# RIKEN-RCCS/GEMMul8

Measured on AMD Instinct MI355X. Metric: emulated DGEMM TFLOPS (N=8192, moduli=14), higher is better.
Workload: dtype int8

## Files before the change

### gemmul8_amd/__init__.py

```python
import ctypes as C
import os

_HERE = os.path.dirname(os.path.abspath(__file__))
LIB_PATH = os.path.join(_HERE, "lib", "libgemmul8.so")

S, D, Cx, Z = 0, 1, 2, 3
INT8, FP8 = 0, 1
OPS = {"N": 0, "T": 1, "C": 2}
UPLO = {"L": 0, "U": 1}
SIDE = {"L": 0, "R": 1}
DIAG = {"N": 0, "U": 1}


class Layout(C.Structure):
    _fields_ = [
        ("kp", C.c_size_t), ("mp", C.c_size_t), ("num_mat", C.c_size_t), ("parts", C.c_size_t),
        ("sizeA", C.c_size_t), ("sizeB", C.c_size_t), ("sizeC", C.c_size_t),
        ("A_lo", C.c_void_p), ("B_lo", C.c_void_p),
        ("part_strideA", C.c_size_t), ("part_strideB", C.c_size_t),
        ("A_bound", C.c_void_p), ("B_bound", C.c_void_p),
        ("sftA", C.c_void_p), ("sftB", C.c_void_p),
        ("C_mid", C.c_void_p), ("scratch", C.c_void_p), ("scratch_bytes", C.c_size_t),
        ("lo_format", C.c_size_t),
    ]


_lib = None

EXPORTS = ["gemmul8_version", "gemmul8_work_size", "gemmul8_gemm", "gemmul8_get_layout", "gemmul8_scale",
           "gemmul8_scale_bounds", "gemmul8_scale_finish", "gemmul8_lowprec_gemm", "gemmul8_crt", "gemmul8_set_fp8_bound_mode", "gemmul8_set_nonfinite_mode",
           "gemmul8_hook_would_emulate", "gemmul8_reload_knobs", "gemmul8_abi_version", "gemmul8_layout_bytes", "gemmul8_syrk", "gemmul8_herk", "gemmul8_syr2k",
           "gemmul8_symm", "gemmul8_hemm", "gemmul8_her2k", "gemmul8_trmm", "gemmul8_trsm", "gemmul8_trsm_work_size", "gemmul8_trsm_leaf"]

ABI_VERSION = 7


def _bind_hip_runtime():
    try:
        import torch
    except Exception:
        pass
    path = None
    with open("/proc/self/maps") as f:
        for line in f:
            if "libamdhip64" in line:
                path = line.split()[-1]
                break
# ... 77 lines not shown
    L.gemmul8_trmm.argtypes = [C.c_void_p, C.c_int, C.c_int, C.c_int, C.c_int, C.c_int, C.c_int, C.c_size_t, C.c_size_t, C.c_void_p, C.c_void_p, C.c_size_t,
                               C.c_void_p, C.c_size_t, C.c_void_p, C.c_size_t, C.c_uint, C.c_int, C.c_void_p, C.POINTER(C.c_double)]
    L.gemmul8_trsm.restype = C.c_int
    L.gemmul8_trsm.argtypes = [C.c_void_p, C.c_int, C.c_int, C.c_int, C.c_int, C.c_int, C.c_int, C.c_size_t, C.c_size_t, C.c_void_p, C.c_void_p, C.c_size_t,
                               C.c_void_p, C.c_size_t, C.c_uint, C.c_int, C.c_void_p, C.POINTER(C.c_double)]
    L.gemmul8_trsm_work_size.restype = C.c_size_t
    L.gemmul8_trsm_work_size.argtypes = [C.c_int, C.c_int, C.c_int, C.c_size_t, C.c_size_t, C.c_uint]
    L.gemmul8_trsm_leaf.restype = C.c_int
    L.gemmul8_trsm_leaf.argtypes = []
    L.gemmul8_set_fp8_bound_mode.restype = C.c_int
    L.gemmul8_set_fp8_bound_mode.argtypes = [C.c_int]
    L.gemmul8_set_nonfinite_mode.restype = C.c_int
    L.gemmul8_set_nonfinite_mode.argtypes = [C.c_int]
    L.gemmul8_hook_would_emulate.restype = C.c_int
    L.gemmul8_hook_would_emulate.argtypes = [C.c_int, C.c_int, C.c_size_t, C.c_size_t, C.c_size_t, C.c_uint, C.c_int, C.c_size_t]
    L.gemmul8_reload_knobs.restype = None
    L.gemmul8_reload_knobs.argtypes = []
    L.gemmul8_add_f64.restype = C.c_int
    L.gemmul8_add_f64.argtypes = [C.c_void_p, C.c_void_p, C.c_void_p, C.c_size_t]
    L.gemmul8_add_row_bias.restype = C.c_int
    L.gemmul8_add_row_bias.argtypes = [C.c_void_p, C.c_int, C.c_size_t, C.c_size_t, C.c_void_p, C.c_size_t, C.c_void_p]
    return L


NONFINITE_REFERENCE, NONFINITE_IEEE = 0, 1


def set_nonfinite_mode(mode):
    prev = lib().gemmul8_set_nonfinite_mode(int(mode))
    if prev < 0:
# ... 308 lines not shown
```

### gemmul8_amd/csrc/oz2_driver.hip

```cpp
#include <hip/hip_runtime.h>
#include <stdint.h>
#include <stdio.h>
#include <stdlib.h>
#include <string.h>

#include <algorithm>

#include <atomic>
#include <mutex>

#include "../../include/gemmul8_c.h"
#include "oz2_gemm_common.hpp"
#include "oz2_kernels.h"
#include "oz2_knobs.hpp"

using namespace oz2;

namespace {

inline char* align256(void* p) {
    uintptr_t x = reinterpret_cast<uintptr_t>(p);
    x = (x + 255) & ~uintptr_t(255);
    return reinterpret_cast<char*>(x);
}
// ... 40 lines not shown
static Knobs parse_knobs() {
    Knobs k;
    auto num = [](const char* name, int dflt) {
        const char* s = getenv(name);
        return s && *s ? atoi(s) : dflt;
    };
    if (const char* e = getenv("GEMMUL8_EPI_NT"); e && (e[0] == '0' || e[0] == '1') && !e[1]) k.epi_nt = e[0] - '0';
    if (const int t = num("GEMMUL8_BOUND_TILE", 0); t == 128 || t == 256) k.bound_tile = t;
    if (num("GEMMUL8_CPLX_BOUND_LAUNCHES", 1) == 2) k.cplx_bound_launches = 2;
    if (const int c = num("GEMMUL8_CPLX_CHUNK", 0); c >= 1) k.cplx_chunk = c;
    if (const char* e = getenv("GEMMUL8_CRT_KERNEL")) k.crt_kernel = e[0] == 'd' ? 1 : e[0] == 'r' ? 2 : 0;
    if (const int c = num("GEMMUL8_GEMM_CUS", 0); c >= 8) k.gemm_cus = c & ~7;
    if (const char* e = getenv("GEMMUL8_FP8_FUSED"); e && e[0] == '0') k.fp8_fused = 0;
    if (const char* e = getenv("GEMMUL8_FP8_PLANES")) k.fp8_planes = e[0] == 'e' ? 1 : 0;
    if (const char* e = getenv("GEMMUL8_SCALE_FOLD"); e && e[0] == '0') k.scale_fold = 0;
    if (const char* e = getenv("GEMMUL8_BOUNDS_ONE_READ"); e && (e[0] == '0' || e[0] == '1') && !e[1]) k.bounds_one_read = e[0] - '0';
    if (const char* e = getenv("GEMMUL8_CRT_PANELS"); e && atoi(e) > 1) {
        k.crt_panels = std::min(atoi(e), 256);
        k.crt_panels_ring = e[strlen(e) - 1] == 'r';
    }
    if (const char* e = getenv("GEMMUL8_MAP_COLBLOCK"); e && *e) k.map_colblock = atoi(e) > 0 ? atoi(e) : 0;
    return k;
}
static std::atomic<const Knobs*> g_knobs{nullptr};
static std::mutex g_knobs_mtx;
void reload_knobs() {
    std::lock_guard<std::mutex> lk(g_knobs_mtx);
    g_knobs.store(new Knobs(parse_knobs()), std::memory_order_release);
}
const Knobs& knobs() {
// ... 208 lines not shown
            OZ2_HIP(launch_gemm_f8_bound_cplx(stream, 3, Ab + 2 * L->sizeA, Bb + 2 * L->sizeB, L->kp, k, m, ncols, fbuf, L->mp, rowmax,
                                              colmax + col_begin));
        } else {
            if (int rc2 = bound_gemm_i8(stream, cplx, L, m, col_end - col_begin, Ab, Bb, rowmax, colmax + col_begin)) return rc2;
        }
    }
    return GEMMUL8_OK;
}

int gemmul8_scale_bounds(void* stream_, int dtype, int backend, int op_A, int op_B, size_t m, size_t n, size_t k, const void* A,
                         size_t lda, const void* B, size_t ldb, unsigned N, size_t col_begin, size_t col_end, const gemmul8_layout* L,
                         int skipA, int skipB) {
    return scale_bounds_nf(stream_, dtype, backend, op_A, op_B, m, n, k, A, lda, B, ldb, N, col_begin, col_end, L, skipA, skipB, false);
}

struct TwinPlanes {
    int8_t* lo;
    size_t plane_stride, part_stride;
};
static int scale_finish_nf(void* stream_, int dtype, int backend, int op_A, int op_B, size_t m, size_t n, size_t k, const void* A, size_t lda,
                           const void* B, size_t ldb, unsigned N, int fastmode, unsigned t_begin, unsigned t_end, const gemmul8_layout* L, int skipA,
                           int skipB, bool nf, const TwinPlanes* twinA = nullptr, const SymSide* sym = nullptr) {
    hipStream_t stream = (hipStream_t)stream_;
    if (!L || !A || !B) return GEMMUL8_E_ARG;
    if (!moduli_ok(dtype, N) || t_end > N || t_begin > t_end) return GEMMUL8_E_NUM_MODULI;
    if (backend == kFP8 && k > 65536) return GEMMUL8_E_ARG;
    op_A = norm_op(op_A);
    op_B = norm_op(op_B);
    if (op_A < 0 || op_A > 2 || op_B < 0 || op_B > 2) return GEMMUL8_E_ARG;
    if (skipA && skipB) return GEMMUL8_OK;
    const bool cplx = is_complex(dtype);
    const bool kmajA = op_A != 0, kmajB = op_B == 0;
    const bool conjA = cplx && op_A == 2, conjB = cplx && op_B == 2;
    QuantOperand oa, ob;
    const bool f6 = backend == kFP8 && L->lo_format == 1;
    if (!skipA) oa = QuantOperand{kmajA, conjA, m, A, lda, L->sftA, (int8_t*)L->A_lo, L->sizeA, L->part_strideA, g_batch.sa, f6 ? L->mp : 0};
    if (!skipB) ob = QuantOperand{kmajB, conjB, n, B, ldb, L->sftB, (int8_t*)L->B_lo, L->sizeB, L->part_strideB, g_batch.sb, f6 ? n : 0};
    oa.nf = ob.nf = nf;
    if (twinA) oa.lo2 = twinA->lo, oa.plane_stride2 = twinA->plane_stride, oa.part_stride2 = twinA->part_stride;
    if (sym) (sym->onB ? ob : oa).sym = sym->form, (sym->onB ? ob : oa).herm = sym->herm;
    if (sym && sym->conj) (sym->onB ? ob : oa).conj = cplx;
    if (fastmode) {
        OZ2_HIP(launch_fast_shift_pair(stream, dtype, backend, N, k, oa, ob));
        if (nf) {
            FlagOperand fa, fb;
            if (!skipA) fa = FlagOperand{kmajA, m, A, lda, g_batch.sa, L->sftA};
            if (!skipB) fb = FlagOperand{kmajB, n, B, ldb, g_batch.sb, L->sftB};
            OZ2_HIP(launch_flag_pair(stream, dtype, k, fa, fb));
        }
    } else {
        int *rowmax, *colmax;
        void* amax;
        int16_t *s0A, *s0B;
        int rc = scale_scratch(L, n, &rowmax, &colmax, &amax, &s0A, &s0B);
        if (rc) return rc;
        if (t_end > t_begin && knobs().scale_fold) {
            const float log2P = backend == kINT8 ? GEMMUL8_LOG2P_INT8[N - 2] : GEMMUL8_LOG2P_FP8[N - 2];
            oa.fin_sft0 = s0A, oa.fin_max = rowmax, oa.fin_log2P = log2P;
            ob.fin_sft0 = s0B, ob.fin_max = colmax, ob.fin_log2P = log2P;
        } else {
            OZ2_HIP(launch_shift_finalize(stream, backend, N, skipA ? 0 : m, rowmax, L->sftA, skipB ? 0 : n, colmax, L->sftB, nf));
        }
    }
    OZ2_HIP(launch_quantise_pair(stream, dtype, backend, (int)t_begin, (int)t_end, k, L->kp, oa, ob));
    return GEMMUL8_OK;
}

int gemmul8_scale_finish(void* stream_, int dtype, int backend, int op_A, int op_B, size_t m, size_t n, size_t k, const void* A,
                         size_t lda, const void* B, size_t ldb, unsigned N, int fastmode, unsigned t_begin, unsigned t_end,
                         const gemmul8_layout* L, int skipA, int skipB) {
    return scale_finish_nf(stream_, dtype, backend, op_A, op_B, m, n, k, A, lda, B, ldb, N, fastmode, t_begin, t_end, L, skipA, skipB, false);
}

static int scale_nf(void* stream_, int dtype, int backend, int op_A, int op_B, size_t m, size_t n, size_t k, const void* A, size_t lda, const void* B,
                    size_t ldb, unsigned N, int fastmode, unsigned t_begin, unsigned t_end, const gemmul8_layout* L, int skipA, int skipB, bool nf,
                    const TwinPlanes* twinA = nullptr, const SymSide* sym = nullptr) {
    if (!fastmode) {
        int rc = scale_bounds_nf(stream_, dtype, backend, op_A, op_B, m, n, k, A, lda, B, ldb, N, 0, n, L, skipA, skipB, nf, sym);
        if (rc) return rc;
    }
    return scale_finish_nf(stream_, dtype, backend, op_A, op_B, m, n, k, A, lda, B, ldb, N, fastmode, t_begin, t_end, L, skipA, skipB, nf, twinA, sym);
}

int gemmul8_scale(void* stream_, int dtype, int backend, int op_A, int op_B, size_t m, size_t n, size_t k, const void* A, size_t lda,
                  const void* B, size_t ldb, unsigned N, int fastmode, unsigned t_begin, unsigned t_end, const gemmul8_layout* L,
                  int skipA, int skipB) {
    return scale_nf(stream_, dtype, backend, op_A, op_B, m, n, k, A, lda, B, ldb, N, fastmode, t_begin, t_end, L, skipA, skipB, false);
}

static int lowprec_gemm_kr(void* stream_, int dtype, int backend, size_t m, size_t n, size_t k, unsigned N, unsigned t_begin, unsigned t_end,
                           const gemmul8_layout* L, int krange) {
    hipStream_t stream = (hipStream_t)stream_;
    if (!L) return GEMMUL8_E_ARG;
    if (krange != 0 && backend != kINT8) return GEMMUL8_E_UNSUPPORTED;
    if (padding256(k) != L->kp) return GEMMUL8_E_ARG;
    if (!moduli_ok(dtype, N) || t_end > N || t_begin > t_end) return GEMMUL8_E_NUM_MODULI;
    const int8_t* A_lo = (const int8_t*)L->A_lo;
    const int8_t* B_lo = (const int8_t*)L->B_lo;
    if (backend == kFP8 && L->lo_format == 1 && n < 64) return GEMMUL8_E_ARG;
    const bool f6 = backend == kFP8 && L->lo_format == 1;
    auto launch_gemm_f8 = [f6](hipStream_t st, int which, const int8_t* A, const int8_t* B, size_t sA, size_t sB, size_t kp, size_t mm, size_t nn, int tb, int te,
                               int16_t* out, size_t ldo, size_t sO, const int16_t* r0, const int16_t* r1, size_t sR, const int16_t* rx = nullptr,
// ... 164 lines not shown
    if (dtype < 0 || dtype > 3 || backend < 0 || backend > 1) return GEMMUL8_E_ARG;
    if (!moduli_ok(dtype, N)) return GEMMUL8_E_NUM_MODULI;
    if (!alpha || !beta || !A || !B || !C || !work) return GEMMUL8_E_ARG;
    if (k > (size_t(1) << 17)) return GEMMUL8_E_ARG;
    if (m == 0 || n == 0 || k == 0) return GEMMUL8_OK;
    gemmul8_layout L;
    int rc = gemmul8_get_layout(dtype, backend, m, n, k, N, work, workA, workB, enA, enB, &L);
    if (rc) return rc;
    const bool skipA = skip_scalA && enA, skipB = skip_scalB && enB;
    Timer* T = timers_ns ? thread_timer() : nullptr;
    if (T && hipEventRecord(T->ev[0], stream) != hipSuccess) {
        (void)hipGetLastError();
        T = nullptr;
    }
    const bool nf = g_nonfinite_mode.load(std::memory_order_relaxed) == 1;
    rc = scale_nf(stream, dtype, backend, op_A, op_B, m, n, k, A, lda, B, ldb, N, fastmode, 0, N, &L, skipA, skipB, nf);
    if (rc) return rc;
    if (T) OZ2_HIP(hipEventRecord(T->ev[1], stream));
    const int P = (backend == kINT8 && !is_complex(dtype) && g_batch.batch <= 1) ? std::min<int>(knobs().crt_panels, (int)((n + 255) / 256)) : 0;
    if (P > 1) {
        const size_t tiles = (n + 255) / 256, esz = is_f32(dtype) ? 4 : 8;
        for (int p = 0; p < P; ++p) {
            const size_t c0 = std::min(n, tiles * p / P * 256), c1 = std::min(n, tiles * (p + 1) / P * 256);
            if (c1 <= c0) continue;
            gemmul8_layout Lp = L;
            Lp.B_lo = (char*)L.B_lo + c0 * L.kp;
            if (!knobs().crt_panels_ring) Lp.C_mid = (char*)L.C_mid + c0 * L.mp;
            rc = gemmul8_lowprec_gemm(stream, dtype, backend, m, c1 - c0, k, N, 0, N, &Lp);
            if (rc) return rc;
            rc = gemmul8_crt(stream, dtype, backend, N, m, c1 - c0, Lp.C_mid, L.mp, L.sizeC, L.sftA, L.sftB + c0, alpha, beta, (char*)C + c0 * ldc * esz, ldc);
            if (rc) return rc;
// ... 527 lines not shown
```

### gemmul8_amd/csrc/oz2_kernels.h

```cpp
#pragma once
#include <hip/hip_runtime.h>
#include <stddef.h>
#include <stdint.h>

#include "oz2_device.hpp"
#include "oz2_knobs.hpp"

namespace oz2 {

enum DType { kF32 = 0, kF64 = 1, kC32 = 2, kC64 = 3 };
inline bool is_complex(int dt) { return dt >= 2; }
inline bool is_f32(int dt) { return dt == kF32 || dt == kC32; }
inline size_t padding256(size_t x) { return (x + 255) / 256 * 256; }
inline unsigned planes_of(int backend, int t) { return backend == kINT8 ? 1u : (t < 6 ? 2u : 3u); }
inline unsigned num_mat(int backend, unsigned N) {
    unsigned s = 0;
    for (unsigned t = 0; t < N; ++t) s += planes_of(backend, (int)t);
    return s;
}
ModTable make_mod_table(int backend);

struct BatchCtx {
    unsigned batch = 1;
    size_t ws = 0;
// ... 63 lines not shown
    size_t xstride = 0;
    size_t f6_rows = 0;
    const int16_t* fin_sft0 = nullptr;
    const int* fin_max = nullptr;
    float fin_log2P = 0.0f;
    bool nf = false;
    int8_t* lo2 = nullptr;
    size_t plane_stride2 = 0, part_stride2 = 0;
    int sym = kSymNone;
    bool herm = false;
};
inline bool f6_planes_ok(size_t n) { return n >= 64 && knobs().fp8_planes != 1; }
hipError_t launch_fast_shift_pair(hipStream_t stream, int dtype, int backend, unsigned N, size_t k, const QuantOperand& A, const QuantOperand& B);
hipError_t launch_quantise_pair(hipStream_t stream, int dtype, int backend, int t_begin, int t_end, size_t k, size_t kp, const QuantOperand& A,
                                const QuantOperand& B);

struct Seg2Planes {
    const void* X2 = nullptr;
    size_t ld2 = 0;
    int8_t* lo2 = nullptr;
    size_t plane_stride2 = 0, part_stride2 = 0;
};
hipError_t launch_fast_shift_seg2(hipStream_t stream, int dtype, unsigned N, size_t k, const QuantOperand& A, const Seg2Planes& S);
hipError_t launch_extract_seg2(hipStream_t stream, int dtype, size_t k, size_t kp, const ExtractOperand& A, const Seg2Planes& S, void* zero_p, size_t zero_bytes);
hipError_t launch_quantise_seg2(hipStream_t stream, int dtype, int t_begin, int t_end, size_t k, size_t kp, const QuantOperand& A, const Seg2Planes& S);

constexpr int16_t kNonfiniteSft = INT16_MIN;
constexpr int kNonfiniteShift = -(int)kNonfiniteSft;
struct FlagOperand {
    bool kmajor = false;
// ... 40 lines not shown
```

### gemmul8_amd/csrc/oz2_knobs.hpp

```cpp
#pragma once

namespace oz2 {

struct Knobs {
    int epi_nt = -1;
    int bound_tile = 0;
    int cplx_bound_launches = 1;
    int cplx_chunk = 0;
    int crt_kernel = 0;
    int fp8_planes = 0;
    int fp8_fused = 1;
    int gemm_cus = 0;
    int crt_panels = 0;
    int crt_panels_ring = 0;
    int scale_fold = 1;
    int bounds_one_read = -1;
    int map_colblock = -1;
};
const Knobs& knobs();
void reload_knobs();

}
```

### gemmul8_amd/csrc/oz2_scale.hip

```cpp
#include <hip/hip_runtime.h>
#include <limits.h>
#include <stdint.h>

#include <algorithm>
#include <type_traits>

#include "oz2_kernels.h"

namespace oz2 {

ModTable make_mod_table(int backend) {
    ModTable T;
    for (int t = 0; t < 20; ++t) {
        const int p = backend == kINT8 ? GEMMUL8_MODULI_INT8[t] : GEMMUL8_MODULI_FP8[t];
        T.mc[t].p = p;
        T.mc[t].invp = 1.0f / (float)p;
        unsigned c[16];
        long long pw = 1;
        for (int i = 0; i < 16; ++i) {
            c[i] = i < 15 ? (unsigned)(pw % p) : 0u;
            pw = (pw % p) * 256;
        }
        for (int i = 0; i < 4; ++i) {
            unsigned lo = 0, hi = 0;
// ... 231 lines not shown
        put_f6_word_f(o + 2 * a.plane_stride, sm);
    }
}

template <bool WIDE> __device__ __forceinline__ int residue_from_small(int Ri, float Rf, const ModConst& mc) {
    const float qf = fmaf(Rf, mc.invp, 12582912.0f);
    int r;
    asm("v_mad_i32_i24 %0, %1, %2, %3" : "=v"(r) : "v"(__float_as_int(qf)), "s"(-mc.p), "v"(Ri));
    if constexpr (WIDE) {
        r += (int)((unsigned)mc.p << 22);
        if (!(mc.p & 1)) r = (r == -(mc.p >> 1)) ? (mc.p >> 1) : r;
    }
    return r;
}

template <typename T, bool TWIN = false, bool SEG2 = false> __device__ __forceinline__ void emit4_mod_float(const StageArgs& a, int8_t* out, [[maybe_unused]] int8_t* out2, const T (&v)[4], int s) {
    using E = ET<T>;
    double xr[4], xi[4];
    bool big = false;
#pragma unroll
    for (int e = 0; e < 4; ++e) {
        xr[e] = trunc(ldexp(E::re(v[e]), s));
        big |= fabs(xr[e]) >= 0x1.0p53;
        if constexpr (E::cplx) {
            xi[e] = trunc(ldexp(E::im(v[e]), s));
            if (a.conj) xi[e] = -xi[e];
            big |= fabs(xi[e]) >= 0x1.0p53;
        } else {
            xi[e] = 0.0;
        }
    }
// ... 81 lines not shown
                        }
                    }
                    if constexpr (SEG2) {
                        int8_t* o2 = out2 + (size_t)tt * a.plane_stride2;
                        *(unsigned*)o2 = pack(rr);
                        if constexpr (E::cplx) {
                            *(unsigned*)(o2 + a.part_stride2) = pack(ri);
                            *(unsigned*)(o2 + 2 * a.part_stride2) = pack(rs);
                        }
                    }
                }
            }
        }
    };
    const bool anybig = __any(big);
    if constexpr (TWIN || SEG2) {
        if (anybig) run.template operator()<false, true>();
        else run.template operator()<false, false>();
        return;
    }
    if (a.backend == kFP8) {
        if (anybig) run.template operator()<true, true>();
        else run.template operator()<true, false>();
    } else {
        if (anybig) run.template operator()<false, true>();
        else run.template operator()<false, false>();
    }
}

template <typename T, int MODE, bool TWIN = false, bool SEG2 = false>
__device__ __forceinline__ void emit4(const StageArgs& a, size_t row, size_t k0, const T (&vin)[4], int s, [[maybe_unused]] unsigned seg = 0) {
    using E = ET<T>;
    if constexpr (SEG2) {
        int8_t* const o1 = a.lo + OZ2_ZW + row * a.pitch + (seg ? a.kp : 0) + k0;
        int8_t* const o2 = a.lo2 + OZ2_ZW + row * a.pitch + (seg ? 0 : a.kp) + k0;
        if constexpr (MODE == MODE_BOUND) {
            unsigned wr = 0, wi = 0, wd = 0;
#pragma unroll
            for (int e = 0; e < 4; ++e) {
                auto ub = [&](double x) { return (int)ceil(ldexp(fabs(x), s)); };
                const int br = ub(E::re(vin[e]));
                wr |= ((unsigned)br & 0xFFu) << (8 * e);
                if constexpr (E::cplx) {
                    const int bi = ub(E::im(vin[e]));
                    wi |= ((unsigned)bi & 0xFFu) << (8 * e);
                    wd |= ((unsigned)(br - bi) & 0xFFu) << (8 * e);
                }
            }
            *(unsigned*)o1 = wr, *(unsigned*)o2 = wr;
            if constexpr (E::cplx) {
                *(unsigned*)(o1 + a.part_stride) = wi, *(unsigned*)(o2 + a.part_stride2) = wi;
                *(unsigned*)(o1 + 2 * a.part_stride) = wd, *(unsigned*)(o2 + 2 * a.part_stride2) = wd;
            }
        } else {
            emit4_mod_float<T, false, true>(a, o1, o2, vin, s);
        }
        return;
    }
    T v[4] = {vin[0], vin[1], vin[2], vin[3]};
    if (MODE == MODE_MOD && a.nf && s == kNonfiniteShift) {
#pragma unroll
        for (int e = 0; e < 4; ++e) v[e] = E::zero();
        s = 0;
    }
    int8_t* out = a.lo + OZ2_ZW + ((MODE == MODE_MOD && a.f6) ? f6_lane_offset(a, row, k0) : row * a.kp + k0);
    if constexpr (MODE == MODE_BOUND) {
        if (a.backend == kFP8) {
            using U = typename E::U;
            unsigned wr = 0, wi = 0, wd = 0;
#pragma unroll
            for (int e = 0; e < 4; ++e) {
// ... 26 lines not shown
                const int bi = ub(E::im(v[e]));
                wi |= ((unsigned)bi & 0xFFu) << (8 * e);
                wd |= ((unsigned)(br - bi) & 0xFFu) << (8 * e);
            }
        }
        *(unsigned*)out = wr;
        if constexpr (E::cplx) {
            *(unsigned*)(out + a.part_stride) = wi;
            *(unsigned*)(out + 2 * a.part_stride) = wd;
        }
    } else {
        emit4_mod_float<T, TWIN>(a, out, TWIN ? a.lo2 + OZ2_ZW + row * a.kp + k0 : nullptr, v, s);
    }
}

template <typename T, int MODE, bool TWIN = false>
__device__ __forceinline__ void stage_kmajor_body(const StageArgs& a, const unsigned bid) {
    using E = ET<T>;
    using U = typename E::U;
    if constexpr (MODE == MODE_MOD) {
        if (a.f6) {
            const unsigned nks = (unsigned)(a.kp / 128);
            const unsigned rg = bid / nks;
            const size_t row = (size_t)rg * 8 + (threadIdx.x >> 5);
            const size_t k0 = (size_t)(bid - rg * nks) * 128 + (size_t)(threadIdx.x & 31) * 4;
            if (row >= a.rows) return;
            const T* x = (const T*)((const char*)a.X + OZ2_ZX) + row * a.ld;
            const int s = OZ2_ROW_SHIFT(a, row, bid == rg * nks && (threadIdx.x & 31) == 0);
            T v[4];
            load4<T>(x, k0, a.k, v);
            emit4<T, MODE, TWIN>(a, row, k0, v, s);
            return;
        }
    }
// ... 144 lines not shown
                T v[4];
                load4<T>(x, k0, a.k, v);
                emit4<T, MODE, false, true>(a, row, k0, v, s, seg);
            }
        }
    }
}

template <typename T> struct StageTile {
#ifndef OZ2_STAGE_TR8
#define OZ2_STAGE_TR8 16
#endif
    static constexpr int TR = sizeof(T) == 4 ? 32 : sizeof(T) == 16 ? 8 : OZ2_STAGE_TR8;
    static constexpr int TK = 128;
};
template <typename T, int MODE, bool TWIN = false, bool SEG2 = false>
__device__ __forceinline__ void stage_strided_body(const StageArgs& a, const unsigned bid) {
    using E = ET<T>;
    using U = typename E::U;
    constexpr int TR = StageTile<T>::TR, TK = StageTile<T>::TK;
    constexpr int PITCH = TK + (sizeof(T) >= 16 ? 1 : 16 / sizeof(T));
    constexpr int CH = TK / 4;
    constexpr int RPP = 256 / CH;
    __shared__ __attribute__((aligned(16))) T tile[TR][PITCH];
    using UBm = typename std::conditional<sizeof(U) == 8, unsigned long long, unsigned>::type;
    [[maybe_unused]] __shared__ UBm rowam[TR];
    const unsigned nrt = (unsigned)((a.rows + TR - 1) / TR);
    const unsigned kt = bid / nrt, rt = bid - kt * nrt;
    const size_t r0 = (size_t)rt * TR;
    [[maybe_unused]] unsigned seg = 0;
    if constexpr (SEG2) seg = kt >= (unsigned)(a.kp / TK);
// ... 68 lines not shown
#pragma unroll 1
    for (int pass = 0; pass < TR / RPP; ++pass) {
        const int rl = pass * RPP + threadIdx.x / CH;
        const size_t row = r0 + rl;
        if (row >= a.rows) continue;
        int s;
        if constexpr (MODE == MODE_BOUND) {
            const UBm bits = rowam[rl];
            U am;
            __builtin_memcpy(&am, &bits, sizeof(U));
            s = (a.backend == kINT8 ? 5 : 7) - ilogb0(am);
            if (kt == 0 && c == 0) {
                ((int16_t*)((char*)a.sft0 + OZ2_ZW))[row] = (int16_t)s;
                if (a.sft0_keep) ((int16_t*)((char*)a.sft0_keep + OZ2_ZW))[row] = (int16_t)s;
            }
        } else {
            s = OZ2_ROW_SHIFT(a, row, kt == 0 && c == 0);
        }
        T v[4];
#pragma unroll
        for (int e = 0; e < 4; ++e) v[e] = tile[rl][c * 4 + e];
        emit4<T, MODE, TWIN, SEG2>(a, row, kb + c * 4, v, s, seg);
    }
}

constexpr int kPanelMaxTiles = 64;
#ifndef OZ2_PANEL_DEPTH
#define OZ2_PANEL_DEPTH 4
#endif
template <typename T> __device__ __forceinline__ void stage_panel_body(const StageArgs& a, const unsigned bid) {
    static_assert(!ET<T>::cplx, "real operands");
    constexpr int TR = StageTile<T>::TR, TK = StageTile<T>::TK;
    constexpr int CH = TK / 4, RPP = 256 / CH, NP = TR / RPP;
    constexpr int RPL = 16 / (int)sizeof(T), RP = TR / RPL, KY = 256 / RP, NL = TK / KY;
    constexpr int D = OZ2_PANEL_DEPTH;
    constexpr int kNone = INT_MIN;
    constexpr int PITCH = TK + 16 / (int)sizeof(T);
// ... 181 lines not shown
    if (km) stage_kmajor_body<T, MODE_MOD, true>(a, blockIdx.x);
    else stage_strided_body<T, MODE_MOD, true>(a, blockIdx.x);
}
template <typename T> __global__ void __launch_bounds__(256) extract_seg2_kernel(const StageArgs a, const int km) {
    if (a.zero_words) {
        unsigned* zp = (unsigned*)((char*)a.zero_p + OZ2_ZW);
        for (unsigned i = blockIdx.x * 256u + threadIdx.x; i < a.zero_words; i += gridDim.x * 256u) zp[i] = 0u;
    }
    if (km) stage_kmajor_seg2_body<T, MODE_BOUND>(a, blockIdx.x);
    else stage_strided_body<T, MODE_BOUND, false, true>(a, blockIdx.x);
}
template <typename T> __global__ void __launch_bounds__(256) quantise_seg2_kernel(const StageArgs a, const int km) {
    if (km) stage_kmajor_seg2_body<T, MODE_MOD>(a, blockIdx.x);
    else stage_strided_body<T, MODE_MOD, false, true>(a, blockIdx.x);
}
static_assert(2 * sizeof(StageArgs) + 16 <= 4096, "two argument blocks must fit the 4 KiB kernel-argument segment");

typedef float v16f __attribute__((ext_vector_type(16)));
typedef unsigned v6u __attribute__((ext_vector_type(6)));
template <typename T> __device__ __forceinline__ void stage_f6_body(const StageArgs& a, const unsigned bid, const bool kmajor, char* tile ) {
    static_assert(!ET<T>::cplx, "real operands");
    constexpr int EPL = 16 / (int)sizeof(T);
    constexpr int CH = 128 / (int)sizeof(T);
    const unsigned lane = threadIdx.x & 63u, q = threadIdx.x >> 6;
    const unsigned nks = (unsigned)(a.kp / 128), nrb = (unsigned)((a.rows + 63) / 64);
    unsigned rb, kt;
    if (kmajor) rb = bid / nks, kt = bid - rb * nks;
    else kt = bid / nrb, rb = bid - kt * nrb;
    const size_t r0 = (size_t)rb * 64, row = r0 + lane, k0 = (size_t)kt * 128 + (size_t)q * 32;
    const T* X = (const T*)((const char*)a.X + OZ2_ZX);
// ... 446 lines not shown
hipError_t launch_extract_seg2(hipStream_t stream, int dtype, size_t k, size_t kp, const ExtractOperand& A, const Seg2Planes& S, void* zero_p, size_t zero_bytes) {
    if (A.one_read || A.conj) return hipErrorInvalidValue;
    StageArgs a = extract_args(kINT8, k, kp, A);
    seg2_args(a, kp, S);
    if (zero_p && zero_bytes) a.zero_p = (unsigned*)zero_p, a.zero_words = (unsigned)(zero_bytes / 4);
    return launch_seg2<MODE_BOUND>(stream, dtype, A.kmajor, a);
}
hipError_t launch_quantise_seg2(hipStream_t stream, int dtype, int t_begin, int t_end, size_t k, size_t kp, const QuantOperand& A, const Seg2Planes& S) {
    if (t_end <= t_begin) return hipSuccess;
    if (A.conj || A.f6_rows || A.nf || A.lo2) return hipErrorInvalidValue;
    StageArgs a = quantise_args(kINT8, t_begin, t_end, k, kp, A);
    seg2_args(a, kp, S);
    return launch_seg2<MODE_MOD>(stream, dtype, A.kmajor, a);
}

hipError_t launch_quantise_pair(hipStream_t stream, int dtype, int backend, int t_begin, int t_end, size_t k, size_t kp, const QuantOperand& A,
                                const QuantOperand& B) {
    if ((A.rows == 0 && B.rows == 0) || t_end <= t_begin) return hipSuccess;
    if (A.sym || B.sym) return launch_quantise_sym_pair(stream, dtype, backend, t_begin, t_end, k, kp, A, B);
    if (A.lo2 || B.lo2) {
        if (B.rows || B.lo2 || A.rows == 0 || !is_complex(dtype) || backend != kINT8 || A.f6_rows || A.nf) return hipErrorInvalidValue;
        return launch_quantise_twin(stream, dtype, t_begin, t_end, k, kp, A);
    }
    const StageArgs a = quantise_args(backend, t_begin, t_end, k, kp, A), b = quantise_args(backend, t_begin, t_end, k, kp, B);
    switch (dtype) {
    case kF32: return launch_quantise_stage<float>(stream, A.kmajor, a, B.kmajor, b);
    case kF64: return launch_quantise_stage<double>(stream, A.kmajor, a, B.kmajor, b);
    case kC32: return launch_quantise_stage<float2>(stream, A.kmajor, a, B.kmajor, b);
    case kC64: return launch_quantise_stage<double2>(stream, A.kmajor, a, B.kmajor, b);
    }
// ... 766 lines not shown
```

### include/gemmul8_c.h

```cpp
#ifndef GEMMUL8_C_H
#define GEMMUL8_C_H

#include <stddef.h>
#include <stdint.h>

#if defined(__GNUC__)
#define GEMMUL8_API __attribute__((visibility("default")))
#else
#define GEMMUL8_API
#endif

#ifdef __cplusplus
extern "C" {
#endif

enum { GEMMUL8_S = 0, GEMMUL8_D = 1, GEMMUL8_C = 2, GEMMUL8_Z = 3 };
enum { GEMMUL8_INT8 = 0, GEMMUL8_FP8 = 1 };
enum { GEMMUL8_OP_N = 0, GEMMUL8_OP_T = 1, GEMMUL8_OP_C = 2 };

enum {
    GEMMUL8_OK = 0,
    GEMMUL8_E_NUM_MODULI = -1,
    GEMMUL8_E_ARG = -2,
    GEMMUL8_E_UNSUPPORTED = -3,
// ... 17 lines not shown
    size_t part_strideA, part_strideB;
    void *A_bound, *B_bound;
    int16_t *sftA, *sftB;
    void *C_mid;
    void *scratch;
    size_t scratch_bytes;
    size_t lo_format;
} gemmul8_layout;

GEMMUL8_API int gemmul8_get_layout(int dtype, int backend, size_t m, size_t n, size_t k, unsigned num_moduli, void *work, void *workA,
                       void *workB, int enable_skip_scalA, int enable_skip_scalB, gemmul8_layout *out);

#define GEMMUL8_ABI_VERSION 7
GEMMUL8_API int gemmul8_abi_version(void);
GEMMUL8_API size_t gemmul8_layout_bytes(void);


GEMMUL8_API int gemmul8_scale(void *stream, int dtype, int backend, int op_A, int op_B, size_t m, size_t n, size_t k, const void *A,
                  size_t lda, const void *B, size_t ldb, unsigned num_moduli, int fastmode, unsigned t_begin,
                  unsigned t_end, const gemmul8_layout *L, int skipA, int skipB);

GEMMUL8_API int gemmul8_scale_bounds(void *stream, int dtype, int backend, int op_A, int op_B, size_t m, size_t n, size_t k,
                                     const void *A, size_t lda, const void *B, size_t ldb, unsigned num_moduli, size_t col_begin,
                                     size_t col_end, const gemmul8_layout *L, int skipA, int skipB);
GEMMUL8_API int gemmul8_scale_finish(void *stream, int dtype, int backend, int op_A, int op_B, size_t m, size_t n, size_t k,
                                     const void *A, size_t lda, const void *B, size_t ldb, unsigned num_moduli, int fastmode,
                                     unsigned t_begin, unsigned t_end, const gemmul8_layout *L, int skipA, int skipB);

GEMMUL8_API int gemmul8_lowprec_gemm(void *stream, int dtype, int backend, size_t m, size_t n, size_t k, unsigned num_moduli,
                         unsigned t_begin, unsigned t_end, const gemmul8_layout *L);
// ... 76 lines not shown
```

Baseline: 159.6.

## Add lean quantise kernels for plain real INT8 GEMM, optionally unpaired launches

Adds a specialised quantise path for plain real f32/f64 INT8 GEMMs. It reads the precomputed shift instead of folding shift finalisation into the quantise kernel, uses a simplified emit path and a 1024-wide k-major chunking. For very large problems it launches separate A and B kernels instead of one paired kernel. The aim is a lighter quantise kernel with fewer registers and branches, at the cost of a separate shift-finalise launch and extra code paths, plus a call counter.

Result: no change. 160.6 (median of 6 runs) (+0.6%).

```diff
diff --git a/gemmul8_amd/__init__.py b/gemmul8_amd/__init__.py
--- a/gemmul8_amd/__init__.py
+++ b/gemmul8_amd/__init__.py
@@ -30,7 +30,7 @@
 EXPORTS = ["gemmul8_version", "gemmul8_work_size", "gemmul8_gemm", "gemmul8_get_layout", "gemmul8_scale",
            "gemmul8_scale_bounds", "gemmul8_scale_finish", "gemmul8_lowprec_gemm", "gemmul8_crt", "gemmul8_set_fp8_bound_mode", "gemmul8_set_nonfinite_mode",
            "gemmul8_hook_would_emulate", "gemmul8_reload_knobs", "gemmul8_abi_version", "gemmul8_layout_bytes", "gemmul8_syrk", "gemmul8_herk", "gemmul8_syr2k",
-           "gemmul8_symm", "gemmul8_hemm", "gemmul8_her2k", "gemmul8_trmm", "gemmul8_trsm", "gemmul8_trsm_work_size", "gemmul8_trsm_leaf"]
+           "gemmul8_symm", "gemmul8_hemm", "gemmul8_her2k", "gemmul8_trmm", "gemmul8_trsm", "gemmul8_trsm_work_size", "gemmul8_trsm_leaf", "gemmul8_scale_lean_rule", "gemmul8_scale_lean_calls"]
 
 ABI_VERSION = 7
 
@@ -138,6 +138,10 @@
     L.gemmul8_set_nonfinite_mode.argtypes = [C.c_int]
     L.gemmul8_hook_would_emulate.restype = C.c_int
     L.gemmul8_hook_would_emulate.argtypes = [C.c_int, C.c_int, C.c_size_t, C.c_size_t, C.c_size_t, C.c_uint, C.c_int, C.c_size_t]
+    L.gemmul8_scale_lean_rule.restype = C.c_int
+    L.gemmul8_scale_lean_rule.argtypes = [C.c_int, C.c_int, C.c_size_t, C.c_size_t, C.c_size_t, C.c_size_t, C.c_int, C.c_int, C.c_int]
+    L.gemmul8_scale_lean_calls.restype = C.c_ulonglong
+    L.gemmul8_scale_lean_calls.argtypes = []
     L.gemmul8_reload_knobs.restype = None
     L.gemmul8_reload_knobs.argtypes = []
     L.gemmul8_add_f64.restype = C.c_int
diff --git a/gemmul8_amd/csrc/oz2_driver.hip b/gemmul8_amd/csrc/oz2_driver.hip
--- a/gemmul8_amd/csrc/oz2_driver.hip
+++ b/gemmul8_amd/csrc/oz2_driver.hip
@@ -78,6 +78,8 @@
     if (const char* e = getenv("GEMMUL8_FP8_FUSED"); e && e[0] == '0') k.fp8_fused = 0;
     if (const char* e = getenv("GEMMUL8_FP8_PLANES")) k.fp8_planes = e[0] == 'e' ? 1 : 0;
     if (const char* e = getenv("GEMMUL8_SCALE_FOLD"); e && e[0] == '0') k.scale_fold = 0;
+    if (const char* e = getenv("GEMMUL8_SCALE_LEAN"); e && (e[0] == '0' || e[0] == '1') && !e[1]) k.scale_lean = e[0] - '0';
+    if (const char* e = getenv("GEMMUL8_SCALE_UNPAIR"); e && (e[0] == '0' || e[0] == '1') && !e[1]) k.scale_unpair = e[0] - '0';
     if (const char* e = getenv("GEMMUL8_BOUNDS_ONE_READ"); e && (e[0] == '0' || e[0] == '1') && !e[1]) k.bounds_one_read = e[0] - '0';
     if (const char* e = getenv("GEMMUL8_CRT_PANELS"); e && atoi(e) > 1) {
         k.crt_panels = std::min(atoi(e), 256);
@@ -316,13 +318,25 @@
     return scale_bounds_nf(stream_, dtype, backend, op_A, op_B, m, n, k, A, lda, B, ldb, N, col_begin, col_end, L, skipA, skipB, false);
 }
 
+constexpr size_t kLeanMinElems = size_t(1) << 24, kLeanUnpairMinElems = size_t(1) << 27;
+int gemmul8_scale_lean_rule(int dtype, int backend, size_t m, size_t n, size_t k, size_t batch, int nonfinite_mode, int caller, int fastmode) {
+    if (dtype != kF32 && dtype != kF64) return 0;
+    if (backend != kINT8 || batch != 1 || nonfinite_mode != 0 || caller != GEMMUL8_CALLER_GEMM) return 0;
+    const size_t elems = (m + n) * padding256(k);
+    if (elems >= kLeanUnpairMinElems) return 2;
+    return !fastmode && elems >= kLeanMinElems ? 1 : 0;
+}
+
+static std::atomic<unsigned long long> g_lean_calls{0};
+unsigned long long gemmul8_scale_lean_calls(void) { return g_lean_calls.load(std::memory_order_relaxed); }
+
 struct TwinPlanes {
     int8_t* lo;
     size_t plane_stride, part_stride;
 };
 static int scale_finish_nf(void* stream_, int dtype, int backend, int op_A, int op_B, size_t m, size_t n, size_t k, const void* A, size_t lda,
                            const void* B, size_t ldb, unsigned N, int fastmode, unsigned t_begin, unsigned t_end, const gemmul8_layout* L, int skipA,
-                           int skipB, bool nf, const TwinPlanes* twinA = nullptr, const SymSide* sym = nullptr) {
+                           int skipB, bool nf, const TwinPlanes* twinA = nullptr, const SymSide* sym = nullptr, bool plain = false) {
     hipStream_t stream = (hipStream_t)stream_;
     if (!L || !A || !B) return GEMMUL8_E_ARG;
     if (!moduli_ok(dtype, N) || t_end > N || t_begin > t_end) return GEMMUL8_E_NUM_MODULI;
@@ -342,6 +356,13 @@
     if (twinA) oa.lo2 = twinA->lo, oa.plane_stride2 = twinA->plane_stride, oa.part_stride2 = twinA->part_stride;
     if (sym) (sym->onB ? ob : oa).sym = sym->form, (sym->onB ? ob : oa).herm = sym->herm;
     if (sym && sym->conj) (sym->onB ? ob : oa).conj = cplx;
+    bool lean = false, unpair = false;
+    if (plain && !twinA && !sym && quantise_lean_ok(dtype, backend, oa, ob)) {
+        const int rule = gemmul8_scale_lean_rule(dtype, backend, m, n, k, g_batch.batch, nf ? 1 : 0, GEMMUL8_CALLER_GEMM, fastmode);
+        const int force = knobs().scale_lean, force2 = knobs().scale_unpair;
+        lean = force < 0 ? rule != 0 : force == 1;
+        unpair = force2 < 0 ? rule == 2 : force2 == 1;
+    }
     if (fastmode) {
         OZ2_HIP(launch_fast_shift_pair(stream, dtype, backend, N, k, oa, ob));
         if (nf) {
@@ -356,7 +377,7 @@
         int16_t *s0A, *s0B;
         int rc = scale_scratch(L, n, &rowmax, &colmax, &amax, &s0A, &s0B);
         if (rc) return rc;
-        if (t_end > t_begin && knobs().scale_fold) {
+        if (t_end > t_begin && knobs().scale_fold && !lean) {
             const float log2P = backend == kINT8 ? GEMMUL8_LOG2P_INT8[N - 2] : GEMMUL8_LOG2P_FP8[N - 2];
             oa.fin_sft0 = s0A, oa.fin_max = rowmax, oa.fin_log2P = log2P;
             ob.fin_sft0 = s0B, ob.fin_max = colmax, ob.fin_log2P = log2P;
@@ -364,30 +385,32 @@
             OZ2_HIP(launch_shift_finalize(stream, backend, N, skipA ? 0 : m, rowmax, L->sftA, skipB ? 0 : n, colmax, L->sftB, nf));
         }
     }
-    OZ2_HIP(launch_quantise_pair(stream, dtype, backend, (int)t_begin, (int)t_end, k, L->kp, oa, ob));
+    if (lean) g_lean_calls.fetch_add(1, std::memory_order_relaxed);
+    if (lean) OZ2_HIP(launch_quantise_lean(stream, dtype, (int)t_begin, (int)t_end, k, L->kp, oa, ob, unpair));
+    else OZ2_HIP(launch_quantise_pair(stream, dtype, backend, (int)t_begin, (int)t_end, k, L->kp, oa, ob));
     return GEMMUL8_OK;
 }
 
 int gemmul8_scale_finish(void* stream_, int dtype, int backend, int op_A, int op_B, size_t m, size_t n, size_t k, const void* A,
                          size_t lda, const void* B, size_t ldb, unsigned N, int fastmode, unsigned t_begin, unsigned t_end,
                          const gemmul8_layout* L, int skipA, int skipB) {
-    return scale_finish_nf(stream_, dtype, backend, op_A, op_B, m, n, k, A, lda, B, ldb, N, fastmode, t_begin, t_end, L, skipA, skipB, false);
+    return scale_finish_nf(stream_, dtype, backend, op_A, op_B, m, n, k, A, lda, B, ldb, N, fastmode, t_begin, t_end, L, skipA, skipB, false, nullptr, nullptr, true);
 }
 
 static int scale_nf(void* stream_, int dtype, int backend, int op_A, int op_B, size_t m, size_t n, size_t k, const void* A, size_t lda, const void* B,
                     size_t ldb, unsigned N, int fastmode, unsigned t_begin, unsigned t_end, const gemmul8_layout* L, int skipA, int skipB, bool nf,
-                    const TwinPlanes* twinA = nullptr, const SymSide* sym = nullptr) {
+                    const TwinPlanes* twinA = nullptr, const SymSide* sym = nullptr, bool plain = false) {
     if (!fastmode) {
         int rc = scale_bounds_nf(stream_, dtype, backend, op_A, op_B, m, n, k, A, lda, B, ldb, N, 0, n, L, skipA, skipB, nf, sym);
         if (rc) return rc;
     }
-    return scale_finish_nf(stream_, dtype, backend, op_A, op_B, m, n, k, A, lda, B, ldb, N, fastmode, t_begin, t_end, L, skipA, skipB, nf, twinA, sym);
+    return scale_finish_nf(stream_, dtype, backend, op_A, op_B, m, n, k, A, lda, B, ldb, N, fastmode, t_begin, t_end, L, skipA, skipB, nf, twinA, sym, plain);
 }
 
 int gemmul8_scale(void* stream_, int dtype, int backend, int op_A, int op_B, size_t m, size_t n, size_t k, const void* A, size_t lda,
                   const void* B, size_t ldb, unsigned N, int fastmode, unsigned t_begin, unsigned t_end, const gemmul8_layout* L,
                   int skipA, int skipB) {
-    return scale_nf(stream_, dtype, backend, op_A, op_B, m, n, k, A, lda, B, ldb, N, fastmode, t_begin, t_end, L, skipA, skipB, false);
+    return scale_nf(stream_, dtype, backend, op_A, op_B, m, n, k, A, lda, B, ldb, N, fastmode, t_begin, t_end, L, skipA, skipB, false, nullptr, nullptr, true);
 }
 
 static int lowprec_gemm_kr(void* stream_, int dtype, int backend, size_t m, size_t n, size_t k, unsigned N, unsigned t_begin, unsigned t_end,
@@ -582,7 +605,7 @@
         T = nullptr;
     }
     const bool nf = g_nonfinite_mode.load(std::memory_order_relaxed) == 1;
-    rc = scale_nf(stream, dtype, backend, op_A, op_B, m, n, k, A, lda, B, ldb, N, fastmode, 0, N, &L, skipA, skipB, nf);
+    rc = scale_nf(stream, dtype, backend, op_A, op_B, m, n, k, A, lda, B, ldb, N, fastmode, 0, N, &L, skipA, skipB, nf, nullptr, nullptr, true);
     if (rc) return rc;
     if (T) OZ2_HIP(hipEventRecord(T->ev[1], stream));
     const int P = (backend == kINT8 && !is_complex(dtype) && g_batch.batch <= 1) ? std::min<int>(knobs().crt_panels, (int)((n + 255) / 256)) : 0;
diff --git a/gemmul8_amd/csrc/oz2_kernels.h b/gemmul8_amd/csrc/oz2_kernels.h
--- a/gemmul8_amd/csrc/oz2_kernels.h
+++ b/gemmul8_amd/csrc/oz2_kernels.h
@@ -101,6 +101,9 @@
 hipError_t launch_fast_shift_pair(hipStream_t stream, int dtype, int backend, unsigned N, size_t k, const QuantOperand& A, const QuantOperand& B);
 hipError_t launch_quantise_pair(hipStream_t stream, int dtype, int backend, int t_begin, int t_end, size_t k, size_t kp, const QuantOperand& A,
                                 const QuantOperand& B);
+bool quantise_lean_ok(int dtype, int backend, const QuantOperand& A, const QuantOperand& B);
+hipError_t launch_quantise_lean(hipStream_t stream, int dtype, int t_begin, int t_end, size_t k, size_t kp, const QuantOperand& A, const QuantOperand& B,
+                                bool unpair);
 
 struct Seg2Planes {
     const void* X2 = nullptr;
diff --git a/gemmul8_amd/csrc/oz2_knobs.hpp b/gemmul8_amd/csrc/oz2_knobs.hpp
--- a/gemmul8_amd/csrc/oz2_knobs.hpp
+++ b/gemmul8_amd/csrc/oz2_knobs.hpp
@@ -14,6 +14,8 @@
     int crt_panels = 0;
     int crt_panels_ring = 0;
     int scale_fold = 1;
+    int scale_lean = -1;
+    int scale_unpair = -1;
     int bounds_one_read = -1;
     int map_colblock = -1;
 };
diff --git a/gemmul8_amd/csrc/oz2_scale.hip b/gemmul8_amd/csrc/oz2_scale.hip
--- a/gemmul8_amd/csrc/oz2_scale.hip
+++ b/gemmul8_amd/csrc/oz2_scale.hip
@@ -269,7 +269,7 @@
     return r;
 }
 
-template <typename T, bool TWIN = false, bool SEG2 = false> __device__ __forceinline__ void emit4_mod_float(const StageArgs& a, int8_t* out, [[maybe_unused]] int8_t* out2, const T (&v)[4], int s) {
+template <typename T, bool TWIN = false, bool SEG2 = false, bool LEAN = false> __device__ __forceinline__ void emit4_mod_float(const StageArgs& a, int8_t* out, [[maybe_unused]] int8_t* out2, const T (&v)[4], int s) {
     using E = ET<T>;
     double xr[4], xi[4];
     bool big = false;
@@ -381,7 +381,7 @@
         }
     };
     const bool anybig = __any(big);
-    if constexpr (TWIN || SEG2) {
+    if constexpr (TWIN || SEG2 || LEAN) {
         if (anybig) run.template operator()<false, true>();
         else run.template operator()<false, false>();
         return;
@@ -395,7 +395,7 @@
     }
 }
 
-template <typename T, int MODE, bool TWIN = false, bool SEG2 = false>
+template <typename T, int MODE, bool TWIN = false, bool SEG2 = false, bool LEAN = false>
 __device__ __forceinline__ void emit4(const StageArgs& a, size_t row, size_t k0, const T (&vin)[4], int s, [[maybe_unused]] unsigned seg = 0) {
     using E = ET<T>;
     if constexpr (SEG2) {
@@ -422,6 +422,11 @@
         } else {
             emit4_mod_float<T, false, true>(a, o1, o2, vin, s);
         }
+        return;
+    }
+    if constexpr (LEAN) {
+        static_assert(MODE == MODE_MOD && !TWIN && !ET<T>::cplx, "the lean form: quantise of a real operand");
+        emit4_mod_float<T, false, false, true>(a, a.lo + row * a.kp + k0, nullptr, vin, s);
         return;
     }
     T v[4] = {vin[0], vin[1], vin[2], vin[3]};
@@ -478,10 +483,22 @@
     }
 }
 
-template <typename T, int MODE, bool TWIN = false>
+template <typename T, int MODE, bool TWIN = false, bool LEAN = false>
 __device__ __forceinline__ void stage_kmajor_body(const StageArgs& a, const unsigned bid) {
     using E = ET<T>;
     using U = typename E::U;
+    if constexpr (LEAN) {
+        static_assert(MODE == MODE_MOD && sizeof(T) <= 8, "the lean form: quantise of a real operand");
+        const unsigned nch = (unsigned)(a.kp / 1024 + (a.kp % 1024 != 0));
+        const size_t row = bid / nch;
+        const size_t k0 = (size_t)(bid - row * nch) * 1024 + (size_t)threadIdx.x * 4;
+        if (k0 >= a.kp) return;
+        const int s = -(int)a.sft[row];
+        T v[4];
+        load4<T>((const T*)a.X + row * a.ld, k0, a.k, v);
+        emit4<T, MODE, false, false, true>(a, row, k0, v, s);
+        return;
+    }
     if constexpr (MODE == MODE_MOD) {
         if (a.f6) {
             const unsigned nks = (unsigned)(a.kp / 128);
@@ -656,7 +673,7 @@
     static constexpr int TR = sizeof(T) == 4 ? 32 : sizeof(T) == 16 ? 8 : OZ2_STAGE_TR8;
     static constexpr int TK = 128;
 };
-template <typename T, int MODE, bool TWIN = false, bool SEG2 = false>
+template <typename T, int MODE, bool TWIN = false, bool SEG2 = false, bool LEAN = false>
 __device__ __forceinline__ void stage_strided_body(const StageArgs& a, const unsigned bid) {
     using E = ET<T>;
     using U = typename E::U;
@@ -755,13 +772,15 @@
                 ((int16_t*)((char*)a.sft0 + OZ2_ZW))[row] = (int16_t)s;
                 if (a.sft0_keep) ((int16_t*)((char*)a.sft0_keep + OZ2_ZW))[row] = (int16_t)s;
             }
+        } else if constexpr (LEAN) {
+            s = -(int)a.sft[row];
         } else {
             s = OZ2_ROW_SHIFT(a, row, kt == 0 && c == 0);
         }
         T v[4];
 #pragma unroll
         for (int e = 0; e < 4; ++e) v[e] = tile[rl][c * 4 + e];
-        emit4<T, MODE, TWIN, SEG2>(a, row, kb + c * 4, v, s, seg);
+        emit4<T, MODE, TWIN, SEG2, LEAN>(a, row, kb + c * 4, v, s, seg);
     }
 }
 
@@ -973,6 +992,17 @@
     if (km) stage_kmajor_seg2_body<T, MODE_MOD>(a, blockIdx.x);
     else stage_strided_body<T, MODE_MOD, false, true>(a, blockIdx.x);
 }
+template <typename T> __global__ void __launch_bounds__(256) quantise_lean_pair_kernel(const StageArgs a, const StageArgs b, const unsigned nA, const int kmA, const int kmB) {
+    if (blockIdx.x < nA) {
+        if (kmA) stage_kmajor_body<T, MODE_MOD, false, true>(a, blockIdx.x);
+        else stage_strided_body<T, MODE_MOD, false, false, true>(a, blockIdx.x);
+    } else {
+        if (kmB) stage_kmajor_body<T, MODE_MOD, false, true>(b, blockIdx.x - nA);
+        else stage_strided_body<T, MODE_MOD, false, false, true>(b, blockIdx.x - nA);
+    }
+}
+template <typename T> __global__ void __launch_bounds__(256) quantise_lean_kmajor_kernel(const StageArgs a) { stage_kmajor_body<T, MODE_MOD, false, true>(a, blockIdx.x); }
+template <typename T> __global__ void __launch_bounds__(256) quantise_lean_strided_kernel(const StageArgs a) { stage_strided_body<T, MODE_MOD, false, false, true>(a, blockIdx.x); }
 static_assert(2 * sizeof(StageArgs) + 16 <= 4096, "two argument blocks must fit the 4 KiB kernel-argument segment");
 
 typedef float v16f __attribute__((ext_vector_type(16)));
@@ -1449,6 +1479,35 @@
     return launch_seg2<MODE_MOD>(stream, dtype, A.kmajor, a);
 }
 
+bool quantise_lean_ok(int dtype, int backend, const QuantOperand& A, const QuantOperand& B) {
+    auto plain = [](const QuantOperand& o) { return !o.conj && !o.f6_rows && !o.fin_max && !o.nf && !o.lo2 && !o.sym && !o.xstride; };
+    return (dtype == kF32 || dtype == kF64) && backend == kINT8 && g_batch.batch == 1 && plain(A) && plain(B);
+}
+template <typename T> static hipError_t launch_quantise_lean_t(hipStream_t stream, bool kmA, const StageArgs& a, bool kmB, const StageArgs& b, bool unpair) {
+    const size_t nA = stage_blocks<T, MODE_MOD>(kmA, a), nB = stage_blocks<T, MODE_MOD>(kmB, b);
+    if (nA > 0x7FFFFFFFull || nB > 0x7FFFFFFFull || (!unpair && nA + nB > 0x7FFFFFFFull)) return hipErrorInvalidConfiguration;
+    if (!unpair) {
+        hipLaunchKernelGGL(quantise_lean_pair_kernel<T>, dim3((unsigned)(nA + nB)), dim3(256), 0, stream, a, b, (unsigned)nA, (int)kmA, (int)kmB);
+        return hipGetLastError();
+    }
+    auto one = [&](bool km, const StageArgs& x, size_t nb) {
+        if (nb == 0) return;
+        if (km) hipLaunchKernelGGL(quantise_lean_kmajor_kernel<T>, dim3((unsigned)nb), dim3(256), 0, stream, x);
+        else hipLaunchKernelGGL(quantise_lean_strided_kernel<T>, dim3((unsigned)nb), dim3(256), 0, stream, x);
+    };
+    one(kmA, a, nA);
+    one(kmB, b, nB);
+    return hipGetLastError();
+}
+hipError_t launch_quantise_lean(hipStream_t stream, int dtype, int t_begin, int t_end, size_t k, size_t kp, const QuantOperand& A, const QuantOperand& B,
+                                bool unpair) {
+    if ((A.rows == 0 && B.rows == 0) || t_end <= t_begin) return hipSuccess;
+    if (!quantise_lean_ok(dtype, kINT8, A, B)) return hipErrorInvalidValue;
+    const StageArgs a = quantise_args(kINT8, t_begin, t_end, k, kp, A), b = quantise_args(kINT8, t_begin, t_end, k, kp, B);
+    return dtype == kF32 ? launch_quantise_lean_t<float>(stream, A.kmajor, a, B.kmajor, b, unpair)
+                         : launch_quantise_lean_t<double>(stream, A.kmajor, a, B.kmajor, b, unpair);
+}
+
 hipError_t launch_quantise_pair(hipStream_t stream, int dtype, int backend, int t_begin, int t_end, size_t k, size_t kp, const QuantOperand& A,
                                 const QuantOperand& B) {
     if ((A.rows == 0 && B.rows == 0) || t_end <= t_begin) return hipSuccess;
diff --git a/include/gemmul8_c.h b/include/gemmul8_c.h
--- a/include/gemmul8_c.h
+++ b/include/gemmul8_c.h
@@ -55,6 +55,10 @@
 #define GEMMUL8_ABI_VERSION 7
 GEMMUL8_API int gemmul8_abi_version(void);
 GEMMUL8_API size_t gemmul8_layout_bytes(void);
+
+enum { GEMMUL8_CALLER_GEMM = 0, GEMMUL8_CALLER_RANK_K = 1, GEMMUL8_CALLER_SYMM = 2, GEMMUL8_CALLER_TRMM = 3, GEMMUL8_CALLER_BATCHED = 4 };
+GEMMUL8_API int gemmul8_scale_lean_rule(int dtype, int backend, size_t m, size_t n, size_t k, size_t batch, int nonfinite_mode, int caller, int fastmode);
+GEMMUL8_API unsigned long long gemmul8_scale_lean_calls(void);
 
 
 GEMMUL8_API int gemmul8_scale(void *stream, int dtype, int backend, int op_A, int op_B, size_t m, size_t n, size_t k, const void *A,
```
